# taithenguyen/ppls

Measured on AMD Instinct MI355X. Metric: accepted subintervals/sec + FP64 F-evals/sec at 1/2/4/8 MI355X, EPSILON=1e-10, higher is better.
Workload: dtype f64

## Files before the change

### ppls_amd/csrc/aq_ring_window.h

```cpp
#pragma once

#if defined(__HIPCC__) || defined(__CUDACC__)
#define AQ_RW_HD __host__ __device__
#else
#define AQ_RW_HD
#endif

namespace aq {

constexpr int RING_CHUNK = 64;

struct RingLines {
    int wcap;
    int line;
    int pf_issue;
    int pf_below;
    int refill;
};

AQ_RW_HD constexpr bool ring_lines_valid(const RingLines& l) {
    return l.wcap >= 2 * RING_CHUNK && l.wcap % RING_CHUNK == 0 &&
           l.line <= l.wcap &&
           l.line >= 2 * RING_CHUNK - 1 &&
           l.pf_below >= 0 && l.pf_below + RING_CHUNK <= l.line &&
           l.pf_issue >= l.pf_below && l.pf_issue < l.line &&
           l.refill >= RING_CHUNK && l.refill % RING_CHUNK == 0 && l.refill <= l.line;
}

AQ_RW_HD constexpr unsigned burst_lo1(const RingLines& l, bool pf_in_flight, bool cellar_nonempty) {
    return (unsigned)(pf_in_flight ? l.pf_below : (cellar_nonempty ? l.pf_issue : 0)) + 1u;
}
AQ_RW_HD constexpr unsigned burst_span(const RingLines& l, unsigned lo1) { return (unsigned)l.line + 1u - lo1; }
AQ_RW_HD constexpr bool above_line(const RingLines& l, unsigned S) { return S > (unsigned)l.line; }
AQ_RW_HD constexpr unsigned exit_chunks(const RingLines& l, unsigned ring, unsigned held) {
    return ring + held > (unsigned)l.wcap
               ? (ring + held - (unsigned)l.wcap + (unsigned)RING_CHUNK - 1u) / (unsigned)RING_CHUNK
               : 0u;
}
AQ_RW_HD constexpr unsigned max_exit_pairs(const RingLines& l) { return (unsigned)l.line + (unsigned)RING_CHUNK; }

}
```

### ppls_amd/csrc/aq_stream.h

```cpp
#pragma once
#include "aq_device.h"
#include "aq_ring_window.h"
#include "aq_shape.h"
#include "aq_xsum.h"

namespace aq {

typedef double f64x2 __attribute__((ext_vector_type(2)));

constexpr int PCAP = 128;
constexpr int DT_STRIDE = 2;
constexpr int LREC = NW * WCAP + PCAP;
constexpr int POOL0 = NW * WCAP;
constexpr int CH = PCAP;
struct DtField {
    unsigned* p;
    __device__ __forceinline__ unsigned& operator[](unsigned j) const { return p[DT_STRIDE * j]; }
    __device__ __forceinline__ DtField operator+(unsigned o) const { return DtField{p + DT_STRIDE * o}; }
};
#ifndef AQ_JOB_RUN_MAX
#define AQ_JOB_RUN_MAX 16
#endif
constexpr int JOB_RUN_MAX = AQ_JOB_RUN_MAX;
#ifndef AQ_GSS_DIV
#define AQ_GSS_DIV 2
#endif
constexpr unsigned GSS_DIV = AQ_GSS_DIV;
#ifndef AQ_HEAP_SEED
#define AQ_HEAP_SEED 1
#endif
constexpr bool HEAP_SEED = AQ_HEAP_SEED != 0;
constexpr int HEAP_D = 4;
constexpr unsigned HEAP_NODES = (2u << HEAP_D) - 1u;
static_assert(HEAP_NODES + 2u <= 64u, "the heap seeding path is one node per lane");
__device__ __forceinline__ unsigned div_small(unsigned q, unsigned nb, float rnb) {
    unsigned d = (unsigned)((float)q * rnb);
    d += (d + 1u) * nb <= q ? 1u : 0u;
    d -= d * nb > q ? 1u : 0u;
    return d;
}
#ifndef AQ_GIVE_MIN
#define AQ_GIVE_MIN 96
#endif
constexpr int GIVE_MIN = AQ_GIVE_MIN;
constexpr int DONATE_MIN = 64;
#ifndef AQ_POLL_ROUNDS
#define AQ_POLL_ROUNDS 256
#endif
constexpr int POLL_ROUNDS = AQ_POLL_ROUNDS;
#ifndef AQ_GIVE_ROUNDS
#define AQ_GIVE_ROUNDS 128
#endif
constexpr int GIVE_ROUNDS = AQ_GIVE_ROUNDS;
#ifndef AQ_SKEWED_GIVE
#define AQ_SKEWED_GIVE 4
#endif
constexpr int SKEWED_GIVE = AQ_SKEWED_GIVE;
#ifndef AQ_SKEWED_POLL
#define AQ_SKEWED_POLL 64
#endif
constexpr int SKEWED_POLL = AQ_SKEWED_POLL;
#ifndef AQ_SKEWED_GIVE_MIN
#define AQ_SKEWED_GIVE_MIN AQ_GIVE_MIN
#endif
constexpr int SKEWED_GIVE_MIN = AQ_SKEWED_GIVE_MIN;
#ifndef AQ_LEAD_SLEEP
#define AQ_LEAD_SLEEP 2
#endif
#ifndef AQ_WIDE_TAB
#define AQ_WIDE_TAB 1
#endif
#ifndef AQ_STAMPS
#define AQ_STAMPS 0
#endif
#ifndef AQ_X_NOFOLD
#define AQ_X_NOFOLD 0
#endif
#ifndef AQ_X_NOCUACC
#define AQ_X_NOCUACC 0
#endif
#ifndef AQ_FLUSHX
#define AQ_FLUSHX 0
#endif
constexpr unsigned LAZY_TICKET = 64;
constexpr unsigned HEAVY_S = 64;
enum : int { ST_ENTRY = 0, ST_INIT, ST_SEED_IN, ST_SEEDED, ST_IDLE, ST_LEAD, ST_BROKE, ST_FLUSHED, ST_EXIT,
             ST_XCC, ST_PRE, ST_CLASS, ST_FEVAL, ST_DONE, ST_KARG, ST_CB, ST_CL, ST_NB, ST_NR, ST_CS, ST_CF,
             ST_CBD, ST_NS, ST_N, ST_STRIDE = 24 };
constexpr int READY_STRIDE = 32;
constexpr int MAXG = 2048;
constexpr unsigned SHARE_ROT = 1021;
constexpr int PCU_ROW = PCU_MAXK - 1;
constexpr unsigned SPAN_BIT = 1u << 31;
constexpr int TAG_SHIFT = 8;
constexpr unsigned TAG_MASK = (1u << 23) - 1u;
__host__ __device__ constexpr unsigned dt_tag(unsigned dt) { return (dt >> TAG_SHIFT) & TAG_MASK; }
static_assert((unsigned)MAXK - 1u <= TAG_MASK, "the tag field must hold every integral of a launch");
__host__ __device__ __forceinline__ size_t parts_row(int slot) { return slot < NPARTS ? (size_t)slot : (size_t)NPARTS; }
#ifndef AQ_TASKS_PER_JOB
#define AQ_TASKS_PER_JOB 120000
#endif
constexpr unsigned TASKS_PER_JOB = AQ_TASKS_PER_JOB;
#ifndef AQ_CCAP
#define AQ_CCAP 2048
#endif
constexpr int CCAP = AQ_CCAP;
#ifndef AQ_FLUSH_LDS
#define AQ_FLUSH_LDS 0
#endif
constexpr bool FLUSH_LDS = AQ_FLUSH_LDS;
#ifndef AQ_SPILL_LINE
#define AQ_SPILL_LINE WCAP
#endif
#ifndef AQ_REFILL
#define AQ_REFILL (WCAP - 64)
#endif
constexpr int REFILL = AQ_REFILL;
#ifndef AQ_PF_BELOW
#define AQ_PF_BELOW (WCAP / 4)
#endif
constexpr int PF_BELOW = AQ_PF_BELOW;
#ifndef AQ_PF_ISSUE
#define AQ_PF_ISSUE 160
#endif
constexpr int PF_ISSUE = AQ_PF_ISSUE;
constexpr RingLines RL{WCAP, AQ_SPILL_LINE, PF_ISSUE, PF_BELOW, REFILL};
static_assert(ring_lines_valid(RL),
              "ring lines: line <= WCAP, a landed prefetch stays at or below the line, a spill finds a whole chunk");
static_assert(exit_chunks(RL, (unsigned)RL.line, 64u) <= 1u && max_exit_pairs(RL) - 64u <= (unsigned)WCAP,
              "a burst's end moves out at most one chunk before it pushes the held pairs back");
static_assert(WCAP / 2 <= PCAP && WCAP / 2 <= CH, "a give or a donation of half a full ring fits the pool / a chunk");
static_assert((AQ_MAX_LEVELS - 1) + (GIVE_ROUNDS > SKEWED_GIVE ? GIVE_ROUNDS : SKEWED_GIVE) < 256,
              "a burst's pairs past the depth cap must not carry the depth byte into the tag");
constexpr int SPILL = RING_CHUNK;

struct alignas(128) Line {
    unsigned v;
    unsigned pad[31];
};

constexpr int NGROUP = 8;
struct QCtl {
    Line tail;
    Line head;
    Line tokens;
    Line jobs;
    Line idle[NGROUP];
    Line done[NGROUP];
};
struct alignas(128) SlotSums {
    unsigned long long tasks, leaves, spilled;
    unsigned levels, error;
    unsigned pcu;
    unsigned win_lo_not, win_hi;
};
struct Ctl {
    SlotSums sums;
    XSum area;
    unsigned long long hist[2 * AQ_MAX_LEVELS];
};

constexpr int CU_BITS = 11;
__host__ __device__ __forceinline__ unsigned long long pack_cu(unsigned long long tasks, unsigned cu) {
    return (tasks << CU_BITS) | (unsigned long long)(cu & ((1u << CU_BITS) - 1u));
}
struct Counts {
    unsigned long long tasks, leaves;
    unsigned levels;
};
__host__ __device__ __forceinline__ Counts slot_counts(const SlotSums& sm, const unsigned long long* wg_words, int grid) {
    Counts c{sm.tasks, sm.leaves, sm.levels};
    if (sm.pcu) {
        for (int w = 0; w < grid; ++w) {
            c.tasks += wg_words[2 * w] >> CU_BITS;
            c.leaves += wg_words[2 * w + 1] >> 8;
            c.levels = max(c.levels, (unsigned)(wg_words[2 * w + 1] & 255u));
        }
    }
    return c;
}

__device__ __forceinline__ int xs_atomic_add(long long* limbs, double x) {
    XDigits g;
    if (!xs_digits(x, g)) return -1;
#pragma unroll
    for (int k = 0; k < 3; ++k)
        if (g.d[k]) atomicAdd(reinterpret_cast<unsigned long long*>(&limbs[g.i + k]), (unsigned long long)g.d[k]);
    return g.i;
}
__device__ __forceinline__ void xs_window_add(SlotSums& sm, int i0, int i1) {
    const int lo = i0 < 0 ? i1 : (i1 < 0 ? i0 : min(i0, i1)), hi = max(i0, i1);
    if (lo < 0) return;
    atomicMax(&sm.win_lo_not, xs_win_lo(lo));
    atomicMax(&sm.win_hi, xs_win_hi(hi));
}

struct Chunk {
    double a[CH], b[CH], fa[CH], fm[CH], fb[CH];
    unsigned dt[CH];
    unsigned count;
    unsigned pad[31];
};

struct CellarChunk {
    f64x2 ab[64], ff[64], fd[64];
};
struct Cellar {
    CellarChunk c[CCAP / 64];
};
// ... 410 lines not shown
        tab[tid].sbits = tv.sbits;
    }
    __syncthreads();
    if constexpr (DIAG) { if (tid == 0) s_dg[DG_T_INIT] = rtc(); }
    stamp(ST_INIT);

    const double eps = P.eps;
    const double eps2 = eps / area_scale<FID>();
    const int max_depth = P.max_depth;
    unsigned shares_main = (unsigned)P.shares;
    int D_main = P.D;
    unsigned long long per_hint = 0;
    if (!PCU && (P.adaptive & 1)) {
        unsigned h = uni(__hip_atomic_load(&P.hint->shares_next, __ATOMIC_RELAXED, __HIP_MEMORY_SCOPE_AGENT));
        if (h) {
            if constexpr (HEAPS) {
                const unsigned long long per =
                    (P.adaptive & 4) ? __hip_atomic_load(&P.hint->per_next, __ATOMIC_RELAXED, __HIP_MEMORY_SCOPE_AGENT)
                                     : (h >= 2u ? (unsigned long long)h * TASKS_PER_JOB : 0ull);
                const unsigned fill = (gridDim.x * (unsigned)NWT + (unsigned)P.nprob - 1u) / (unsigned)P.nprob;
                const unsigned long long cap = per / MIN_JOB_TASKS;
                h = uni(max(h, (unsigned)min((unsigned long long)fill, cap)));
                per_hint = per;
            }
            shares_main = h;
            D_main = seed_depth_job((unsigned long long)h * (unsigned long long)P.nshards);
        }
    }
    const unsigned W = gridDim.x * (unsigned)NWT;
    const unsigned w_all = bid * (unsigned)NWT + wid;
    const unsigned grp = bid % (unsigned)NGROUP;
    const unsigned grp_size = (gridDim.x - grp + (unsigned)NGROUP - 1u) / (unsigned)NGROUP;
    const int t0 = (int)min(gridDim.x, (unsigned)NGROUP);
    const unsigned tail_from = (!PCU && shares_main >= 8u) ? (unsigned)P.tail_from : (unsigned)P.nprob;
    const unsigned shares_tail = min(shares_main * (unsigned)P.tail_mult, W);
    const int D_tail = seed_depth_job((unsigned long long)shares_tail * (unsigned long long)P.nshards);
    const unsigned main_jobs = tail_from * shares_main;
    const unsigned total_jobs = main_jobs + ((unsigned)P.nprob - tail_from) * shares_tail;
    const unsigned base = wid * WCAP;
    long long* const xs_a = reinterpret_cast<long long*>(s_a + base + (WCAP - 64));
    long long* const xs_b = reinterpret_cast<long long*>(s_b + base + (WCAP - 64));
    const unsigned ring8 = pr_base + base * 8u;
    __builtin_assume((ring8 & (unsigned)(WCAP * 8 - 1)) == 0u);
    unsigned ring_vmask = (unsigned)((WCAP - 1) << 3);
    asm volatile("" : "+v"(ring_vmask));

    Acc acc{0.0, 0.0, 0u, 0u, 0u, 0u, 0u, 0u};
    ErrAcc<ERR> eacc;
    auto err_leaf = [&](double d) {
        if constexpr (ERR) {
            eacc.sg += d / area_scale<FID>();
            eacc.ab += fabs(d) / area_scale<FID>();
        }
    };
    int tag = 0;
    Theta<FID> th{};
    sload_theta<FID>(th, P.theta, tag);
    unsigned ctop = 0;
    Cellar* __restrict__ cel = P.cellar + w_all;
    const bool static_jobs = PCU || P.static_jobs != 0;
    unsigned job = (static_jobs || HEAPS) ? wid * gridDim.x + bid : w_all;
    bool job_pending = false;
    unsigned claim = 0;
    unsigned jpc = (!static_jobs && shares_main == 1u && P.nshards == 1 && JOB_RUN_MAX > 1)
                       ? max(1u, min((unsigned)JOB_RUN_MAX, total_jobs / (4u * W)))
                       : 1u;
    if constexpr (HEAPS) {
        if (per_hint) jpc = uni(max(1u, min(jpc, (unsigned)min((unsigned long long)TASKS_PER_JOB / per_hint, 64ull))));
    }
    unsigned job_end = job + 1u;
    unsigned claim_n = jpc;
    unsigned err = 0;
    bool mixed = false;
    unsigned top = 0, bot = 0;
    bool counted_idle = false;
    bool fresh = true;
    constexpr unsigned give_rounds = FID == F_SIN_RECIP ? (unsigned)SKEWED_GIVE : (unsigned)GIVE_ROUNDS;
    constexpr unsigned poll_rounds = FID == F_SIN_RECIP ? (unsigned)SKEWED_POLL : (unsigned)POLL_ROUNDS;
    constexpr unsigned give_min = FID == F_SIN_RECIP ? (unsigned)SKEWED_GIVE_MIN : (unsigned)GIVE_MIN;
    unsigned poll_ctr = wid * (poll_rounds / NWT);
    unsigned seen_head = 0, seen_tail = 0;
    unsigned long long spilled = 0;
    unsigned long long lock_spins = 0;
    unsigned pf_n = 0;
    PairRegs pf{};
    unsigned long long cl0 = 0;
    if constexpr (DIAG) {
        if (tid == 0) s_dg[DG_T_START] = t_entry;
        cl0 = clk();
    }
    if constexpr (AQ_STAMPS && !DIAG) cl0 = clk();

    auto spill_to_cellar = [&](unsigned b, unsigned c) {
        for (unsigned q = 0; q < (unsigned)SPILL; q += 64u) {
            PairRegs r;
            lds_issue6(ring_addr(ring8, ring_slot(b + q) + lane, ring_vmask), r);
            lds_wait6(r);
            chunk_store(&cel->c[(c + q) / 64u], lane, r);
        }
        if constexpr (DIAG) {
            if (lane == 0) {
                atomicAdd(&s_dg[DG_CELLAR_OUT], (unsigned long long)SPILL);
                atomicMax(&s_dg[DG_MAX_CELLAR], (unsigned long long)(c + SPILL));
            }
        }
    };
    auto chunk_out = [&](unsigned& bt, unsigned& ct, unsigned& pfn) {
        if (pfn) {
            ct += pfn;
            pfn = 0;
        }
        if (ct + (unsigned)SPILL <= (unsigned)CCAP) {
            spill_to_cellar(bt, ct);
            ct += (unsigned)SPILL;
            bt += (unsigned)SPILL;
            return;
        }
        wave_lock(&S.lock, lane, lock_spins);
        const unsigned pt = uni(S.ptop);
        const bool fits = (pt - S.pbot) + 64u <= (unsigned)PCAP;
        if (fits) {
            copy_pair(R, base + ring_slot(bt + lane), POOL0 + ((pt + lane) & (PCAP - 1)));
            if (lane == 0) S.ptop = pt + 64u;
        }
        wave_unlock(&S.lock, lane);
        if (!fits) {
            unsigned slot = 0;
            if (lane == 0) {
                slot = g_add(&qc->tail.v, 1u);
                if (slot < P.qcap) g_add((int*)&qc->tokens.v, 64 + 1);
                spilled += 64;
            }
            slot = uni(__shfl(slot, 0, 64));
            if (slot < P.qcap) {
                const unsigned b = bt;
                publish_chunk(P, R, slot, 64u, [&](unsigned i) { return base + ring_slot(b + i); }, lane);
            } else {
                err |= ERRB_OVERFLOW;
            }
        }
        if constexpr (DIAG) { if (lane == 0) atomicAdd(&s_dg[DG_POOL_PUSH], 64ull); }
        bt += 64;
    };
    const ExpConsts kk = pinned_exp_consts();
    constexpr bool burst_cap = !HIST;
    for (;;) {
        top = uni(top);
        bot = uni(bot);
        ctop = uni(ctop);
        pf_n = uni(pf_n);
        poll_ctr = uni(poll_ctr);
        if (pf_n && top - bot <= (unsigned)PF_BELOW) {
            if (bot < 64u) {
                bot += (unsigned)WCAP;
                top += (unsigned)WCAP;
            }
            bot -= pf_n;
            if (lane < pf_n) lds_store6(ring_addr(ring8, ring_slot(bot) + lane, ring_vmask), pf);
            if constexpr (DIAG) { if (lane == 0) atomicAdd(&s_dg[DG_PREFETCH], (unsigned long long)pf_n); }
            __builtin_amdgcn_wave_barrier();
            pf_n = 0;
        }
        unsigned size = top - bot;

        if (size == 0) {
            if (ctop > 0) {
                unsigned long long cr = 0;
                if constexpr (DIAG) cr = clk();
                const unsigned k = min(ctop, (unsigned)REFILL), c0 = ctop - k;
                for (unsigned q = 0; q < k; q += 64)
                    lds_store6(ring_addr(ring8, q + lane, ring_vmask), chunk_load(&cel->c[(c0 + q) / 64u], lane));
                ctop = c0;
                bot = 0;
                top = k;
                if constexpr (DIAG) {
                    if (lane == 0) {
                        atomicAdd(&s_dg[DG_CELLAR_IN], (unsigned long long)k);
                        atomicAdd(&s_dg[DG_C_REFILL], clk() - cr);
                    }
                }
                __builtin_amdgcn_wave_barrier();
                continue;
            }
            unsigned long long ci = 0;
            if constexpr (DIAG) ci = clk();
            if (counted_idle) {
                const unsigned pt = uni(__hip_atomic_load(&S.ptop, __ATOMIC_RELAXED, __HIP_MEMORY_SCOPE_WORKGROUP));
                const unsigned pb = uni(__hip_atomic_load(&S.pbot, __ATOMIC_RELAXED, __HIP_MEMORY_SCOPE_WORKGROUP));
                const int ph = uni(__hip_atomic_load(&S.phase, __ATOMIC_RELAXED, __HIP_MEMORY_SCOPE_WORKGROUP));
                if (pt == pb) {
                    if (ph == 2) break;
                    __builtin_amdgcn_s_sleep(4);
                    if constexpr (DIAG) { if (lane == 0) atomicAdd(&s_dg[DG_C_IDLE], clk() - ci); }
                    __builtin_amdgcn_wave_barrier();
                    continue;
                }
            }
            if (job_pending) {
                job = W + uni(__shfl(claim, 0, 64));
                job_end = job + claim_n;
                job_pending = false;

            }
            unsigned k = 0;
            int ptag = 0;
            bool lead = false, seed = false;
            int phase = 0;
            bool counted_now = false;
            const bool pool_empty = uni(__hip_atomic_load(&S.ptop, __ATOMIC_RELAXED, __HIP_MEMORY_SCOPE_WORKGROUP)) ==
                                    uni(__hip_atomic_load(&S.pbot, __ATOMIC_RELAXED, __HIP_MEMORY_SCOPE_WORKGROUP));
            if (job < total_jobs && (fresh || pool_empty)) {
                seed = true;
            } else if (!counted_idle && !job_pending && job >= total_jobs && pool_empty) {
                stamp(ST_IDLE);
                unsigned old = 0;
                if (lane == 0) old = __hip_atomic_fetch_add(&S.idle, 1, __ATOMIC_RELAXED, __HIP_MEMORY_SCOPE_WORKGROUP);
                old = uni(__shfl(old, 0, 64));
                counted_idle = true;
                counted_now = old + 1u != (unsigned)NWT;
            }
            if (!seed && !counted_now) {
                wave_lock(&S.lock, lane, lock_spins);
                {
                    const unsigned avail = uni(S.ptop - S.pbot);
                    phase = uni(S.phase);
                    if (avail > 0) {
                        k = min(avail, (unsigned)REFILL);
                        const unsigned pb = S.pbot;
                        ptag = (int)uni(dt_tag(s_dt[POOL0 + (pb & (PCAP - 1))]));
                        for (unsigned q0 = 0; q0 < k; q0 += 64) {
                            const unsigned q = q0 + lane;
                            const unsigned long long bad =
                                __ballot(q < k && (int)dt_tag(s_dt[POOL0 + ((pb + q) & (PCAP - 1))]) != ptag);
                            if (bad) {
                                k = q0 + (unsigned)__builtin_ctzll(bad);
                                break;
                            }
                        }
                        for (unsigned i = lane; i < k; i += 64) copy_pair(R, POOL0 + ((pb + i) & (PCAP - 1)), base + i);
                        if (lane == 0) {
                            S.pbot = pb + k;
                            if (counted_idle) __hip_atomic_fetch_add(&S.idle, -1, __ATOMIC_RELAXED, __HIP_MEMORY_SCOPE_WORKGROUP);
                        }
                        __builtin_amdgcn_wave_barrier();
                        counted_idle = false;
// ... 484 lines not shown
            }
            flush_acc<FID, PCU, ERR>(P, acc, tag, lane, S, s_pc, s_wdd + wid, NWT, xs_a, xs_b, eacc, s_werr + wid);
            if (lane == 0) {
                if (!last) {
                    bool ended = false;
                    if constexpr (PCU) {
                        for (unsigned spins = 0; spins < LAZY_TICKET; ++spins) {
                            if (ld_wt(&qc->done[grp].v)) { ended = true; break; }
                            __builtin_amdgcn_s_sleep(AQ_LEAD_SLEEP);
                        }
                    }
                    if (ended) cmd = -1;
                    const unsigned h = ended ? 0u : g_add(&qc->head.v, 1u);
                    unsigned long long t_prog = rtc();
                    int seen_tk = 0;
                    unsigned seen_tl = ~0u;
                    for (unsigned spins = 0; !ended; ++spins) {
                        const unsigned rv = h < P.qcap ? ld_wt(&P.ready[(size_t)h * READY_STRIDE]) : 0u;
                        const unsigned dn = ld_wt(&qc->done[grp].v);
                        if (rv == P.epoch) { cmd = (int)h; break; }
                        if (dn) { cmd = -1; break; }
                        if ((spins & 63u) == 63u) {
                            const int tk = g_ld((int*)&qc->tokens.v);
                            const unsigned tl = g_ld(&qc->tail.v);
                            const unsigned long long now = rtc();
                            if (tk != seen_tk || tl != seen_tl) {
                                seen_tk = tk;
                                seen_tl = tl;
                                t_prog = now;
                            } else if (now - t_prog > P.stall_ticks) {
                                err |= ERRB_TIMEOUT;
                                cmd = -2;
                                break;
                            }
                        }
                        __builtin_amdgcn_s_sleep(AQ_LEAD_SLEEP);
                    }
                }
                if (cmd >= 0) {
                    __builtin_amdgcn_fence(__ATOMIC_ACQUIRE, "wavefront");
                    cnt = ld_wt(&P.chunks[cmd].count);
                }
            }
            cmd = uni(__shfl(cmd, 0, 64));
            cnt = uni(__shfl(cnt, 0, 64));
            if constexpr (DIAG) { if (lane == 0 && cmd < 0) atomicMax(&s_dg[DG_T_DONE], rtc()); }
            if (cmd < 0) stamp(ST_DONE);
            if (cmd < 0) {
                if (lane == 0) __hip_atomic_store(&S.phase, 2, __ATOMIC_RELAXED, __HIP_MEMORY_SCOPE_WORKGROUP);
                __builtin_amdgcn_wave_barrier();
                break;
            }
            const Chunk* __restrict__ c = P.chunks + cmd;
            wave_lock(&S.lock, lane, lock_spins);
            const unsigned pt = uni(S.ptop);
            for (unsigned i = lane; i < cnt; i += 64) {
                const unsigned j = POOL0 + ((pt + i) & (PCAP - 1));
                s_a[j] = ld_wt(&c->a[i]); s_b[j] = ld_wt(&c->b[i]);
                s_fa[j] = ld_wt(&c->fa[i]); s_fm[j] = ld_wt(&c->fm[i]); s_fb[j] = ld_wt(&c->fb[i]);
                s_dt[j] = ld_wt(&c->dt[i]);
            }
            if (lane == 0) {
                S.ptop = pt + cnt;
                S.phase = 0;
                S.busy_token = 1;
                __hip_atomic_fetch_add(&S.idle, -1, __ATOMIC_RELAXED, __HIP_MEMORY_SCOPE_WORKGROUP);
                const bool was_all_idle = g_add(&qc->idle[grp].v, ~0u) == grp_size;
                g_add((int*)&qc->tokens.v, (was_all_idle ? 1 : 0) - (int)(cnt + 1u));
            }
            counted_idle = false;
            wave_unlock(&S.lock, lane);
            if constexpr (DIAG) {
                if (lane == 0) {
                    atomicAdd(&s_dg[DG_CHUNKS_IN], 1ull);
                    atomicAdd(&s_dg[DG_RECORDS_IN], (unsigned long long)cnt);
                    atomicAdd(&s_dg[DG_T_WAIT], rtc() - tl);
                }
            }
            __builtin_amdgcn_wave_barrier();
            continue;
        }

        if (above_line(RL, size)) {
            chunk_out(bot, ctop, pf_n);
            __builtin_amdgcn_wave_barrier();
            continue;
        }

        ++poll_ctr;
        if ((poll_ctr % poll_rounds) == 0) {
            unsigned slot = 0xffffffffu;
            if (lane == 0) {
                if constexpr (DIAG) atomicAdd(&s_dg[DG_POLLS], 1ull);
                if ((int)(seen_head - seen_tail) > 0) {
                    unsigned expect = seen_tail;
                    if (__hip_atomic_compare_exchange_strong(&qc->tail.v, &expect, seen_tail + 1u, __ATOMIC_RELAXED,
                                                             __ATOMIC_RELAXED, __HIP_MEMORY_SCOPE_AGENT))
                        slot = seen_tail;
                    if constexpr (DIAG) atomicAdd(&s_dg[DG_POLLS], 1ull << 32);
                }
                seen_head = g_ld(&qc->head.v);
                seen_tail = g_ld(&qc->tail.v);
            }
            slot = uni(__shfl(slot, 0, 64));
            if (slot != 0xffffffffu) {
                if (slot >= P.qcap) {
                    err |= ERRB_OVERFLOW;
                } else {
                    wave_lock(&S.lock, lane, lock_spins);
                    const unsigned pavail = uni(S.ptop - S.pbot);
                    unsigned k;
                    if (pavail >= (unsigned)DONATE_MIN) {
                        k = min((unsigned)CH, pavail / 2u);
                        const unsigned pb = S.pbot;
                        if (lane == 0) g_add((int*)&qc->tokens.v, (int)k + 1);
                        publish_chunk(P, R, slot, k, [&](unsigned i) { return POOL0 + ((pb + i) & (PCAP - 1)); }, lane);
                        if (lane == 0) S.pbot = pb + k;
                        wave_unlock(&S.lock, lane);
                    } else {
                        wave_unlock(&S.lock, lane);
                        k = size / 2u;
                        if (lane == 0) g_add((int*)&qc->tokens.v, (int)k + 1);
                        const unsigned b = bot;
                        publish_chunk(P, R, slot, k, [&](unsigned i) { return base + ring_slot(b + i); }, lane);
                        bot += k;
                    }
                    if (lane == 0) spilled += k;
                    if constexpr (DIAG) {
                        if (lane == 0) {
                            atomicAdd(&s_dg[DG_CHUNKS_OUT], 1ull);
                            atomicAdd(&s_dg[DG_RECORDS_OUT], (unsigned long long)k);
                        }
                    }
                    __builtin_amdgcn_wave_barrier();
                    continue;
                }
            }
        }

        if ((poll_ctr % give_rounds) == 0 && size >= give_min &&
            uni(__hip_atomic_load(&S.idle, __ATOMIC_RELAXED, __HIP_MEMORY_SCOPE_WORKGROUP)) > 0 &&
            uni(__hip_atomic_load(&S.ptop, __ATOMIC_RELAXED, __HIP_MEMORY_SCOPE_WORKGROUP)) ==
                uni(__hip_atomic_load(&S.pbot, __ATOMIC_RELAXED, __HIP_MEMORY_SCOPE_WORKGROUP))) {
            const unsigned k = size / 2u;
            wave_lock(&S.lock, lane, lock_spins);
            const unsigned pt = uni(S.ptop);
            const bool fits = (pt - S.pbot) + k <= (unsigned)PCAP;
            if (fits) {
                for (unsigned i = lane; i < k; i += 64)
                    copy_pair(R, base + ring_slot(bot + i), POOL0 + ((pt + i) & (PCAP - 1)));
                if (lane == 0) S.ptop = pt + k;
            }
            wave_unlock(&S.lock, lane);
            if constexpr (DIAG) { if (lane == 0) atomicAdd(&s_dg[DG_GIVE], (unsigned long long)(fits ? k : 0u)); }
            if (fits) {
                bot += k;
                __builtin_amdgcn_wave_barrier();
                continue;
            }
        }
        if (ctop > 0 && pf_n == 0 && size <= (unsigned)PF_ISSUE) {
            pf_n = 64u;
            ctop -= pf_n;
            pf = chunk_load(&cel->c[ctop / 64u], lane);
            __builtin_amdgcn_wave_barrier();
        }

        unsigned long long cb0 = 0;
        if constexpr (AQ_STAMPS && !DIAG) cb0 = clk();
        unsigned b_top = uni(top), b_size = uni(size), b_poll = uni(poll_ctr);
        unsigned b_n = 0;
        unsigned long long b_dv = 0;
        unsigned b_bot = uni(bot), b_ctop = uni(ctop), b_pf = uni(pf_n);
        bool b_mixed = uni(mixed);
        unsigned b_S = b_size, b_S0 = b_size;
        unsigned long long b_am = 0;
        double ca = 0.0, cb = 0.0, cfa = 0.0, cfm = 0.0, cfb = 0.0, cdw = 0.0;
        unsigned b_lo1, b_span;
        auto window = [&]() {
            b_lo1 = burst_lo1(RL, b_pf != 0u, b_ctop > 0u);
            b_span = burst_span(RL, b_lo1);
        };
        window();
        constexpr bool prio_by_load = PCU && FID == F_SIN_RECIP;
        const bool b_heavy = prio_by_load && b_S >= HEAVY_S;
        const unsigned b_max = give_rounds - b_poll % give_rounds;
        unsigned b_rem = b_max;
        __builtin_amdgcn_s_waitcnt(0xC07F);
        bool b_go;
        for (;;) {
        for (;;) {
            unsigned long long c0 = 0, c1 = 0;
            if constexpr (DIAG) c0 = clk();
            if constexpr (prio_by_load) {
                if (b_heavy) asm volatile("s_setprio 3");
                else asm volatile("s_setprio 1");
            }
            const unsigned long long need = ~b_am;
            const unsigned k = min((unsigned)__popcll(need), b_top - b_bot);
            const unsigned jr = mbcnt(need);
            const unsigned long long fmsk = __ballot(jr < k) & need;
            b_top -= k;
            const unsigned paddr = ring_addr(ring8, ring_slot(b_top) + jr, ring_vmask);
            lds_pop6_masked(fmsk, paddr, paddr + 3u * 50u * 512u, ca, cb, cfa, cfm, cfb, cdw);
            const unsigned long long am = b_am | fmsk;
            const unsigned na = (unsigned)__popcll(am);
            const double pa = ca, pb = cb, pfa = cfa, pfm = cfm, pfb = cfb;
            const unsigned long long dtw = (unsigned long long)__double_as_longlong(cdw);
            const unsigned dt = (unsigned)dtw;
            using StepT = typename std::conditional<ERR, Step2e, Step2>::type;
            StepT st[2];
            unsigned long long nospan = 0ull;
            if constexpr (FID == F_COSH4) nospan = __ballot((int)dt >= 0);
            double pm, hm;
            pair_step_halves<FID, WIDE ? 255u : 127u, StepT>(pa, pb, pfa, pfm, pfb, eps2, tab, st, pm, hm, kk,
                                                              FID == F_COSH4 ? 2 : -1, nospan & am, th);
            if constexpr (prio_by_load) { if (!b_heavy) asm volatile("s_setprio 0"); }
            const unsigned long long r0m = __ballot(st[0].refine), r1m = __ballot(st[1].refine);
            unsigned long long okm = am;
            if constexpr (!burst_cap) {
                const unsigned long long dm = __ballot((dt & 255u) < (unsigned)(max_depth - 1));
                okm = am & dm;
                const unsigned long long atcap = am & ~dm;
                if (__builtin_expect(atcap != 0ull, 0)) b_dv |= atcap & (r0m | r1m);
            }
            const unsigned long long l0m = am & ~r0m, l1m = am & ~r1m;
            b_n += na;
            const unsigned long long mask0 = okm & r0m, mask1 = okm & r1m;
            const unsigned cdt = dt + 1u;
            const unsigned long long cdtw = ((dtw >> 32) << 32) | (unsigned long long)cdt;
            masked_acc3(acc.r, st[0].area2, l0m, st[1].area2, l1m, acc.maxdt, burst_cap ? cdt : dt,
                        burst_cap ? (mask0 | mask1) : am);
            if constexpr (ERR) masked_err4(eacc.sg, eacc.ab, st[0].diff, l0m, st[1].diff, l1m);
            if constexpr (DIAG) {
                const int rtag = (int)dt_tag(dt);
                b_mixed |= (__ballot(rtag != tag) & am) != 0ull;
            }
            if (HIST) {
                const unsigned d = dt & 255u;
                if (__builtin_amdgcn_inverse_ballot_w64(am)) {
                    atomicAdd(&P.ctls[P.first_slot + tag].hist[d], 2ull);
                    const unsigned nl = ((l0m >> lane) & 1u) + ((l1m >> lane) & 1u);
                    if (nl) atomicAdd(&P.ctls[P.first_slot + tag].hist[AQ_MAX_LEVELS + d], (unsigned long long)nl);
                }
            }
            if constexpr (DIAG) c1 = clk();
            lds_push6_masked(mask1, ring_addr(ring8, ring_slot(b_top) + mbcnt(mask1), ring_vmask), hm, pb, pfm,
                             st[1].fmid, pfb, __longlong_as_double((long long)cdtw));
            b_top += (unsigned)__popcll(mask1);
            cb = hm;
            cfb = pfm;
            cfm = st[0].fmid;
            cdw = __longlong_as_double((long long)cdtw);
            b_am = mask0;
            if constexpr (DIAG) {
                if (lane == 0) {
                    const unsigned long long c2 = clk();
                    atomicAdd(&s_dg[DG_ROUNDS], 1ull);
                    atomicAdd(&s_dg[DG_ACTIVE_LANES], (unsigned long long)na);
                    atomicAdd(&s_dg[DG_C_ROUND], c2 - c0);
                    atomicAdd(&s_dg[DG_C_EVAL], c1 - c0);
                    atomicMax(&s_dg[DG_MAX_RING], (unsigned long long)b_S);
                    atomicMax(&s_dg[DG_T_LAST_ROUND], rtc());
                    atomicAdd(&s_dg[DG_ACTIVE_TASKS], 2ull * na);
                }
            }
            b_S = (b_top - b_bot) + (unsigned)__popcll(mask0);
            --b_rem;
            unsigned span_r = b_rem != 0u ? b_span : 0u;
            asm("" : "+s"(span_r));
            b_go = b_S - b_lo1 < span_r;
            __builtin_amdgcn_wave_barrier();
            if (!b_go) break;
        }
            unsigned b_re = b_rem;
            asm volatile("" : "+s"(b_re));
            const unsigned sz = b_S;
            if (b_re != 0u && sz != 0u) {
                if (above_line(RL, sz)) {
                    if (b_pf) {
                        b_ctop += b_pf;
                        b_pf = 0;
                    }
                    if (b_ctop + (unsigned)SPILL <= (unsigned)CCAP) {
                        spill_to_cellar(b_bot, b_ctop);
                        b_ctop += (unsigned)SPILL;
                        b_bot += (unsigned)SPILL;
                        b_S -= (unsigned)SPILL;
                        b_S0 -= (unsigned)SPILL;
                        b_go = true;
                    }
                } else if (b_pf) {
                    if (b_bot < 64u) {
                        b_bot += (unsigned)WCAP;
                        b_top += (unsigned)WCAP;
                    }
                    b_bot -= b_pf;
                    if (lane < b_pf) lds_store6(ring_addr(ring8, ring_slot(b_bot) + lane, ring_vmask), pf);
                    if constexpr (DIAG) { if (lane == 0) atomicAdd(&s_dg[DG_PREFETCH], (unsigned long long)b_pf); }
                    b_S += b_pf;
                    b_S0 += b_pf;
                    b_pf = 0;
                    b_go = true;
                } else if (b_ctop > 0u) {
                    b_pf = 64u;
                    b_ctop -= 64u;
                    pf = chunk_load(&cel->c[b_ctop / 64u], lane);
                    b_go = true;
                }
                if (b_go) window();
            }
            __builtin_amdgcn_wave_barrier();
            if (!b_go) break;
        }
        if constexpr (prio_by_load) asm volatile("s_setprio 0");
        bool b_capped = false;
        if constexpr (burst_cap) b_capped = __ballot((acc.maxdt & 255u) >= (unsigned)max_depth) != 0ull;
        if (!__builtin_expect(b_capped, 0)) {
            for (unsigned n = uni(exit_chunks(RL, b_top - b_bot, (unsigned)__popcll(b_am))); n != 0u; --n) {
                chunk_out(b_bot, b_ctop, b_pf);
                b_S0 -= 64u;
            }
        }
        lds_push6_masked(b_am, ring_addr(ring8, ring_slot(b_top) + mbcnt(b_am), ring_vmask), ca, cb, cfa, cfm, cfb,
                         cdw);
        b_top += (unsigned)__popcll(b_am);
        bot = b_bot;
        ctop = b_ctop;
        pf_n = b_pf;
        b_poll += (b_max - b_rem) - 1u;
        top = b_top;
        poll_ctr = b_poll;
        acc.ut += 2u * b_n;
        acc.ul += b_n - ((b_top - b_bot) - b_S0);
        dd_add(acc.hi, acc.lo, acc.r);
        acc.r = 0.0;
        if (b_dv) err |= ERRB_DEPTH;
        if constexpr (burst_cap) {
            if (__builtin_expect(b_capped, 0)) {
                err |= ERRB_DEPTH;
                top = bot;
                ctop = 0;
                pf_n = 0;
            }
        }
        mixed = b_mixed;
        if constexpr (AQ_STAMPS && !DIAG) {
            stp[ST_CB] += clk() - cb0;
            stp[ST_NB] += 1ull;
            stp[ST_NR] += (unsigned long long)(b_max - b_rem);
        }
        __builtin_amdgcn_wave_barrier();
    }

    if constexpr (DIAG) { if (lane == 0) atomicMax(&s_dg[DG_T_BROKE], rtc()); }
    stamp(ST_BROKE);
    flush_acc<FID, PCU, ERR>(P, acc, tag, lane, S, s_pc, s_wdd + wid, NWT, xs_a, xs_b, eacc, s_werr + wid);
    if constexpr (DIAG) { if (lane == 0) atomicMax(&s_dg[DG_T_FLUSHED], rtc()); }
    stamp(ST_FLUSHED);
    if (mixed) err |= ERRB_OVERFLOW;
    const unsigned werr = wave_or_full(err);
    unsigned last_u = 0;
    if (lane == 0) {
        if (werr) {
            for (int p = 0; p < P.nprob; ++p)
                atomicOr(&P.ctls[P.first_slot + p].sums.error, werr);
        }
        if (spilled) atomicAdd(&P.ctls[P.first_slot].sums.spilled, spilled);
        if constexpr (DIAG) {
            atomicAdd(&s_dg[DG_LOCK_SPINS], lock_spins);
            atomicAdd(&s_dg[DG_SPILL_RECORDS], spilled);
            atomicAdd(&s_dg[DG_C_LOOP], clk() - cl0);
        }
        __builtin_amdgcn_fence(__ATOMIC_RELEASE, "workgroup");
        const bool last = atomicAdd(&S.exited, 1u) == (unsigned)NWT - 1u;
        __builtin_amdgcn_fence(__ATOMIC_ACQUIRE, "workgroup");
        last_u = last ? 1u : 0u;
        if (last) {
            const unsigned long long wt = __hip_atomic_load(&S.tasks, __ATOMIC_RELAXED, __HIP_MEMORY_SCOPE_WORKGROUP);
            if (wt && !AQ_X_NOCUACC) __hip_atomic_fetch_add(&P.cu_acc[cu_slot()], wt, __ATOMIC_RELAXED, __HIP_MEMORY_SCOPE_AGENT);
        }
        if constexpr (DIAG) { if (last) atomicMax(&s_dg[DG_T_FOLD], rtc()); }
        if (PCU && last) {
            const unsigned cu = cu_slot();
            for (int p = 0; p < P.nprob; ++p) {
                const unsigned long long t = __hip_atomic_load(&s_pc[p], __ATOMIC_RELAXED, __HIP_MEMORY_SCOPE_WORKGROUP);
                const unsigned long long l = __hip_atomic_load(&s_pc[PCU_ROW + p], __ATOMIC_RELAXED, __HIP_MEMORY_SCOPE_WORKGROUP);
                const unsigned m = (unsigned)__hip_atomic_load(&s_pc[2 * PCU_ROW + p], __ATOMIC_RELAXED, __HIP_MEMORY_SCOPE_WORKGROUP);
                unsigned long long* wp = P.parts + 2 * ((size_t)p * gridDim.x + bid);
                wp[0] = pack_cu(t, cu);
                wp[1] = (l << 8) | (unsigned long long)(m & 255u);
                if (bid == 0) {
                    SlotSums& sm = P.ctls[P.first_slot + p].sums;
                    sm.pcu = 1u;
                    sm.win_lo_not = xs_win_lo(0);
                    sm.win_hi = (unsigned)XS_LIMBS;
                }
            }
        }
        if (!PCU && last && (P.adaptive & 2)) {
            const unsigned long long wt = __hip_atomic_load(&S.tasks, __ATOMIC_RELAXED, __HIP_MEMORY_SCOPE_WORKGROUP);
            __hip_atomic_fetch_add(&P.hint->tasks, wt, __ATOMIC_RELAXED, __HIP_MEMORY_SCOPE_AGENT);
            const unsigned g = __hip_atomic_fetch_add(&P.hint->exits, 1u, __ATOMIC_ACQ_REL, __HIP_MEMORY_SCOPE_AGENT);
            if (g == gridDim.x - 1u) {
                const unsigned long long tot = __hip_atomic_load(&P.hint->tasks, __ATOMIC_ACQUIRE, __HIP_MEMORY_SCOPE_AGENT);
                const unsigned long long per = tot / (unsigned long long)P.nprob;
                unsigned long long sh = (per + TASKS_PER_JOB / 2) / TASKS_PER_JOB;
                sh = sh < 1ull ? 1ull : (sh > (unsigned long long)W ? (unsigned long long)W : sh);
                __hip_atomic_store(&P.hint->shares_next, (unsigned)sh, __ATOMIC_RELAXED, __HIP_MEMORY_SCOPE_AGENT);
                if constexpr (HEAPS) __hip_atomic_store(&P.hint->per_next, per, __ATOMIC_RELAXED, __HIP_MEMORY_SCOPE_AGENT);
                __hip_atomic_store(&P.hint->tasks, 0ull, __ATOMIC_RELAXED, __HIP_MEMORY_SCOPE_AGENT);
                __hip_atomic_store(&P.hint->exits, 0u, __ATOMIC_RELAXED, __HIP_MEMORY_SCOPE_AGENT);
            }
        }
    }
    if constexpr (PCU && !AQ_X_NOFOLD) {
        if (uni(__shfl(last_u, 0, 64))) {
            for (int p = 0; p < P.nprob; ++p) {
                double hi = 0.0, lo = 0.0;
                if (lane < (unsigned)NWT) {
                    const double2 w = s_wdd[p * NWT + (int)lane];
                    hi = w.x;
                    lo = w.y;
                }
                row_sum_dd(hi, lo);
                if (lane == 0) {
// ... 48 lines not shown
```

Measured before the change: 315.7 billion.

## Spill ring chunks to cellar mid-burst so bursts need not stop at the line

Adds a push line (default WCAP-1). When the cellar has room, the burst span is left open instead of being capped at the spill line. Before each push that would exceed the push line, the bottom chunk of the LDS ring is spilled to the cellar inside the round, with any in-flight prefetch first folded into the cellar top. The aim is to avoid ending bursts early and paying the exit/re-entry overhead, at the cost of extra spill traffic and logic inside the hot loop.

```diff
diff --git a/ppls_amd/csrc/aq_ring_window.h b/ppls_amd/csrc/aq_ring_window.h
--- a/ppls_amd/csrc/aq_ring_window.h
+++ b/ppls_amd/csrc/aq_ring_window.h
@@ -39,4 +39,22 @@
 }
 AQ_RW_HD constexpr unsigned max_exit_pairs(const RingLines& l) { return (unsigned)l.line + (unsigned)RING_CHUNK; }
 
+AQ_RW_HD constexpr bool push_line_valid(const RingLines& l, int push) {
+    return push == 0 || (push <= l.wcap - 1 &&
+                         push >= 2 * RING_CHUNK - 1 &&
+                         l.pf_below + RING_CHUNK <= push);
 }
+AQ_RW_HD constexpr bool cellar_room(unsigned ctop, unsigned pf, unsigned ccap) { return ctop + pf + (unsigned)RING_CHUNK <= ccap; }
+constexpr unsigned BURST_SPAN_OPEN = 1u << 30;
+AQ_RW_HD constexpr unsigned burst_span_push(const RingLines& l, int push, unsigned lo1, bool room) {
+    return push != 0 && room ? BURST_SPAN_OPEN : burst_span(l, lo1);
+}
+AQ_RW_HD constexpr bool push_spills(int push, unsigned ring_filled, unsigned pushes) {
+    return push != 0 && ring_filled + pushes > (unsigned)push;
+}
+AQ_RW_HD constexpr unsigned max_round_pairs(const RingLines& l, int push) {
+    return push != 0 && (unsigned)push + (unsigned)RING_CHUNK > (unsigned)l.line ? (unsigned)push + (unsigned)RING_CHUNK
+                                                                                  : (unsigned)l.line;
+}
+
+}
diff --git a/ppls_amd/csrc/aq_stream.h b/ppls_amd/csrc/aq_stream.h
--- a/ppls_amd/csrc/aq_stream.h
+++ b/ppls_amd/csrc/aq_stream.h
@@ -124,7 +124,14 @@
 #define AQ_PF_ISSUE 160
 #endif
 constexpr int PF_ISSUE = AQ_PF_ISSUE;
+#ifndef AQ_PUSH_LINE
+#define AQ_PUSH_LINE (WCAP - 1)
+#endif
+constexpr int PUSH_LINE = AQ_PUSH_LINE;
 constexpr RingLines RL{WCAP, AQ_SPILL_LINE, PF_ISSUE, PF_BELOW, REFILL};
+static_assert(push_line_valid(RL, PUSH_LINE),
+              "push line: <= WCAP - 1, an in-round spill finds a whole chunk, a landing stays at or below it");
+static_assert(CCAP % RING_CHUNK == 0 && CCAP >= RING_CHUNK, "the cellar holds whole chunks");
 static_assert(ring_lines_valid(RL),
               "ring lines: line <= WCAP, a landed prefetch stays at or below the line, a spill finds a whole chunk");
 static_assert(exit_chunks(RL, (unsigned)RL.line, 64u) <= 1u && max_exit_pairs(RL) - 64u <= (unsigned)WCAP,
@@ -1527,7 +1534,7 @@
         unsigned b_lo1, b_span;
         auto window = [&]() {
             b_lo1 = burst_lo1(RL, b_pf != 0u, b_ctop > 0u);
-            b_span = burst_span(RL, b_lo1);
+            b_span = burst_span_push(RL, PUSH_LINE, b_lo1, cellar_room(b_ctop, b_pf, (unsigned)CCAP));
         };
         window();
         constexpr bool prio_by_load = PCU && FID == F_SIN_RECIP;
@@ -1593,9 +1600,24 @@
                 }
             }
             if constexpr (DIAG) c1 = clk();
+            const unsigned np1 = (unsigned)__popcll(mask1);
+            if constexpr (PUSH_LINE != 0) {
+                if (__builtin_expect(push_spills(PUSH_LINE, b_top - b_bot, np1), 0)) {
+                    if (cellar_room(b_ctop, b_pf, (unsigned)CCAP)) {
+                        b_ctop += b_pf;
+                        b_pf = 0;
+                        spill_to_cellar(b_bot, b_ctop);
+                        b_ctop += (unsigned)SPILL;
+                        b_bot += (unsigned)SPILL;
+                        b_S0 -= (unsigned)SPILL;
+                        window();
+                    }
+                    __builtin_amdgcn_wave_barrier();
+                }
+            }
             lds_push6_masked(mask1, ring_addr(ring8, ring_slot(b_top) + mbcnt(mask1), ring_vmask), hm, pb, pfm,
                              st[1].fmid, pfb, __longlong_as_double((long long)cdtw));
-            b_top += (unsigned)__popcll(mask1);
+            b_top += np1;
             cb = hm;
             cfb = pfm;
             cfm = st[0].fmid;
```

Result: no change. 316.1 billion, median of 6 (+0.1%).

## Replace deferred cellar prefetch with synchronous chunk refill into the ring

Applied to the files above, without the earlier changes.

Removes the two-phase cellar prefetch, where a chunk was loaded into registers and landed in the LDS ring later. A single chunk_in now loads from global memory and stores straight into the ring. The issue threshold is set equal to the landing threshold, and the pf register state is dropped from the burst loop and chunk_out. This cuts register pressure and control flow, but the global-load latency is no longer hidden behind compute. The change also adds optional per-event timing stamps (spill, refill, end-of-burst chunk out) behind AQ_STAMPS, with ST_STRIDE widened to 32.

```diff
diff --git a/ppls_amd/csrc/aq_stream.h b/ppls_amd/csrc/aq_stream.h
--- a/ppls_amd/csrc/aq_stream.h
+++ b/ppls_amd/csrc/aq_stream.h
@@ -86,7 +86,9 @@
 constexpr unsigned HEAVY_S = 64;
 enum : int { ST_ENTRY = 0, ST_INIT, ST_SEED_IN, ST_SEEDED, ST_IDLE, ST_LEAD, ST_BROKE, ST_FLUSHED, ST_EXIT,
              ST_XCC, ST_PRE, ST_CLASS, ST_FEVAL, ST_DONE, ST_KARG, ST_CB, ST_CL, ST_NB, ST_NR, ST_CS, ST_CF,
-             ST_CBD, ST_NS, ST_N, ST_STRIDE = 24 };
+             ST_CBD, ST_NS,
+             ST_EV_C, ST_EV_N = ST_EV_C + 3, ST_N = ST_EV_N + 3, ST_STRIDE = 32 };
+enum : int { EV_SPILL = 0, EV_REFILL, EV_END };
 constexpr int READY_STRIDE = 32;
 constexpr int MAXG = 2048;
 constexpr unsigned SHARE_ROT = 1021;
@@ -121,9 +123,10 @@
 #endif
 constexpr int PF_BELOW = AQ_PF_BELOW;
 #ifndef AQ_PF_ISSUE
-#define AQ_PF_ISSUE 160
+#define AQ_PF_ISSUE (WCAP / 4)
 #endif
 constexpr int PF_ISSUE = AQ_PF_ISSUE;
+static_assert(PF_ISSUE == PF_BELOW, "the refill is issued and landed in one event: one line");
 constexpr RingLines RL{WCAP, AQ_SPILL_LINE, PF_ISSUE, PF_BELOW, REFILL};
 static_assert(ring_lines_valid(RL),
               "ring lines: line <= WCAP, a landed prefetch stays at or below the line, a spill finds a whole chunk");
@@ -701,8 +704,6 @@
     unsigned seen_head = 0, seen_tail = 0;
     unsigned long long spilled = 0;
     unsigned long long lock_spins = 0;
-    unsigned pf_n = 0;
-    PairRegs pf{};
     unsigned long long cl0 = 0;
     if constexpr (DIAG) {
         if (tid == 0) s_dg[DG_T_START] = t_entry;
@@ -724,11 +725,7 @@
             }
         }
     };
-    auto chunk_out = [&](unsigned& bt, unsigned& ct, unsigned& pfn) {
-        if (pfn) {
-            ct += pfn;
-            pfn = 0;
-        }
+    auto chunk_out = [&](unsigned& bt, unsigned& ct) {
         if (ct + (unsigned)SPILL <= (unsigned)CCAP) {
             spill_to_cellar(bt, ct);
             ct += (unsigned)SPILL;
@@ -761,25 +758,23 @@
         if constexpr (DIAG) { if (lane == 0) atomicAdd(&s_dg[DG_POOL_PUSH], 64ull); }
         bt += 64;
     };
+    auto chunk_in = [&](unsigned& bt, unsigned& tp, unsigned& ct) {
+        if (bt < 64u) {
+            bt += (unsigned)WCAP;
+            tp += (unsigned)WCAP;
+        }
+        bt -= 64u;
+        ct -= 64u;
+        lds_store6(ring_addr(ring8, ring_slot(bt) + lane, ring_vmask), chunk_load(&cel->c[ct / 64u], lane));
+        if constexpr (DIAG) { if (lane == 0) atomicAdd(&s_dg[DG_PREFETCH], 64ull); }
+    };
     const ExpConsts kk = pinned_exp_consts();
     constexpr bool burst_cap = !HIST;
     for (;;) {
         top = uni(top);
         bot = uni(bot);
         ctop = uni(ctop);
-        pf_n = uni(pf_n);
         poll_ctr = uni(poll_ctr);
-        if (pf_n && top - bot <= (unsigned)PF_BELOW) {
-            if (bot < 64u) {
-                bot += (unsigned)WCAP;
-                top += (unsigned)WCAP;
-            }
-            bot -= pf_n;
-            if (lane < pf_n) lds_store6(ring_addr(ring8, ring_slot(bot) + lane, ring_vmask), pf);
-            if constexpr (DIAG) { if (lane == 0) atomicAdd(&s_dg[DG_PREFETCH], (unsigned long long)pf_n); }
-            __builtin_amdgcn_wave_barrier();
-            pf_n = 0;
-        }
         unsigned size = top - bot;
 
         if (size == 0) {
@@ -1430,7 +1425,7 @@
         }
 
         if (above_line(RL, size)) {
-            chunk_out(bot, ctop, pf_n);
+            chunk_out(bot, ctop);
             __builtin_amdgcn_wave_barrier();
             continue;
         }
@@ -1507,10 +1502,9 @@
                 continue;
             }
         }
-        if (ctop > 0 && pf_n == 0 && size <= (unsigned)PF_ISSUE) {
-            pf_n = 64u;
-            ctop -= pf_n;
-            pf = chunk_load(&cel->c[ctop / 64u], lane);
+        if (ctop > 0 && size <= (unsigned)PF_BELOW) {
+            chunk_in(bot, top, ctop);
+            size += 64u;
             __builtin_amdgcn_wave_barrier();
         }
 
@@ -1519,14 +1513,14 @@
         unsigned b_top = uni(top), b_size = uni(size), b_poll = uni(poll_ctr);
         unsigned b_n = 0;
         unsigned long long b_dv = 0;
-        unsigned b_bot = uni(bot), b_ctop = uni(ctop), b_pf = uni(pf_n);
+        unsigned b_bot = uni(bot), b_ctop = uni(ctop);
         bool b_mixed = uni(mixed);
         unsigned b_S = b_size, b_S0 = b_size;
         unsigned long long b_am = 0;
         double ca = 0.0, cb = 0.0, cfa = 0.0, cfm = 0.0, cfb = 0.0, cdw = 0.0;
         unsigned b_lo1, b_span;
         auto window = [&]() {
-            b_lo1 = burst_lo1(RL, b_pf != 0u, b_ctop > 0u);
+            b_lo1 = burst_lo1(RL, false, b_ctop > 0u);
             b_span = burst_span(RL, b_lo1);
         };
         window();
@@ -1537,6 +1531,7 @@
         __builtin_amdgcn_s_waitcnt(0xC07F);
         bool b_go;
         for (;;) {
+        asm volatile("" : "+s"(b_rem));
         for (;;) {
             unsigned long long c0 = 0, c1 = 0;
             if constexpr (DIAG) c0 = clk();
@@ -1625,11 +1620,10 @@
             asm volatile("" : "+s"(b_re));
             const unsigned sz = b_S;
             if (b_re != 0u && sz != 0u) {
+                unsigned long long ce0 = 0;
+                int ev = -1;
+                if constexpr (AQ_STAMPS && !DIAG) ce0 = clk();
                 if (above_line(RL, sz)) {
-                    if (b_pf) {
-                        b_ctop += b_pf;
-                        b_pf = 0;
-                    }
                     if (b_ctop + (unsigned)SPILL <= (unsigned)CCAP) {
                         spill_to_cellar(b_bot, b_ctop);
                         b_ctop += (unsigned)SPILL;
@@ -1637,26 +1631,25 @@
                         b_S -= (unsigned)SPILL;
                         b_S0 -= (unsigned)SPILL;
                         b_go = true;
-                    }
-                } else if (b_pf) {
-                    if (b_bot < 64u) {
-                        b_bot += (unsigned)WCAP;
-                        b_top += (unsigned)WCAP;
-                    }
-                    b_bot -= b_pf;
-                    if (lane < b_pf) lds_store6(ring_addr(ring8, ring_slot(b_bot) + lane, ring_vmask), pf);
-                    if constexpr (DIAG) { if (lane == 0) atomicAdd(&s_dg[DG_PREFETCH], (unsigned long long)b_pf); }
-                    b_S += b_pf;
-                    b_S0 += b_pf;
-                    b_pf = 0;
+                        ev = EV_SPILL;
+                    }
+                } else if (b_ctop > 0u) {
+                    chunk_in(b_bot, b_top, b_ctop);
+                    b_S += 64u;
+                    b_S0 += 64u;
                     b_go = true;
-                } else if (b_ctop > 0u) {
-                    b_pf = 64u;
-                    b_ctop -= 64u;
-                    pf = chunk_load(&cel->c[b_ctop / 64u], lane);
-                    b_go = true;
+                    ev = EV_REFILL;
                 }
                 if (b_go) window();
+                if constexpr (AQ_STAMPS && !DIAG) {
+                    if (ev >= 0) {
+                        const unsigned long long dc = clk() - ce0;
+                        for (int i = 0; i < EV_END; ++i) {
+                            stp[ST_EV_C + i] += ev == i ? dc : 0ull;
+                            stp[ST_EV_N + i] += ev == i ? 1ull : 0ull;
+                        }
+                    }
+                }
             }
             __builtin_amdgcn_wave_barrier();
             if (!b_go) break;
@@ -1666,8 +1659,14 @@
         if constexpr (burst_cap) b_capped = __ballot((acc.maxdt & 255u) >= (unsigned)max_depth) != 0ull;
         if (!__builtin_expect(b_capped, 0)) {
             for (unsigned n = uni(exit_chunks(RL, b_top - b_bot, (unsigned)__popcll(b_am))); n != 0u; --n) {
-                chunk_out(b_bot, b_ctop, b_pf);
+                unsigned long long ce0 = 0;
+                if constexpr (AQ_STAMPS && !DIAG) ce0 = clk();
+                chunk_out(b_bot, b_ctop);
                 b_S0 -= 64u;
+                if constexpr (AQ_STAMPS && !DIAG) {
+                    stp[ST_EV_C + EV_END] += clk() - ce0;
+                    stp[ST_EV_N + EV_END] += 1ull;
+                }
             }
         }
         lds_push6_masked(b_am, ring_addr(ring8, ring_slot(b_top) + mbcnt(b_am), ring_vmask), ca, cb, cfa, cfm, cfb,
@@ -1675,7 +1674,6 @@
         b_top += (unsigned)__popcll(b_am);
         bot = b_bot;
         ctop = b_ctop;
-        pf_n = b_pf;
         b_poll += (b_max - b_rem) - 1u;
         top = b_top;
         poll_ctr = b_poll;
@@ -1689,7 +1687,6 @@
                 err |= ERRB_DEPTH;
                 top = bot;
                 ctop = 0;
-                pf_n = 0;
             }
         }
         mixed = b_mixed;
```

Result: no change. 315.4 billion before, 317.5 billion after, median of 6 (+0.6%).
